# ayankele/dune-transformercvn

Hardware: AMD Instinct MI355X
Metric: events/sec (fwd+bwd) at batch=32, 8 prongs/event; fraction of MFMA roofline (higher is better)
Workload: dtype bf16; 1 GPU; TransformerCVN DenseNet [3,6,12,6,3] g32, fwd+loss+bwd, batch 32/GPU, 8 prongs/event, 3x400x280 maps, 6-layer encoder, dropout 0.1; global_batch=32, parallelism=dp1, precision=bf16

## Files before the change

dune-transformercvn_amd/csrc/densenet.hip:

```cpp
#include <string>
#include <vector>
#include <cstring>

#include "tcvn_rows.h"
#include <cstdlib>
#include "densenet_plan.h"

using namespace tcvn;

namespace {
constexpr float kEps = 1e-5f, kMom = 0.1f;
}

int DenseNetPlan::add_slot(const std::string& name, long numel, int kind) {
    slots.push_back({name, numel, kind});
    return (int)slots.size() - 1;
}
BnSlots DenseNetPlan::add_bn(const std::string& p, int c) {
    BnSlots s;
    s.w = add_slot(p + ".weight", c, TCVN_SLOT_PARAM);
    s.b = add_slot(p + ".bias", c, TCVN_SLOT_PARAM);
    s.rm = add_slot(p + ".running_mean", c, TCVN_SLOT_BUFFER);
    s.rv = add_slot(p + ".running_var", c, TCVN_SLOT_BUFFER);
    s.nbt = add_slot(p + ".num_batches_tracked", 1, TCVN_SLOT_COUNTER);
// ... 490 lines not shown
    const int mid = cfg.bn_size * cfg.growth, g = cfg.growth;
    char* D = s.ws + L.D[bi];
    char* Y = s.ws + L.Y[bi][l];
    double* bstatD = reinterpret_cast<double*>(s.ws + L.bstatD[bi]);
    double* bstatY = reinterpret_cast<double*>(s.ws + L.bstatY[bi][l]);
    long long* isumD = s.lf_on ? reinterpret_cast<long long*>(s.ws + L.isumD[bi]) : nullptr;
    long long* isumY = s.lf_on ? reinterpret_cast<long long*>(s.ws + L.isumY[bi][l]) : nullptr;
    int rc;
    ConvFwdArgs a = conv3_args(s, bi, l);
    Fwd1x1Args f1;
    const LayerPath p = path[bi][l] = layer_path(s, bi, l, a, f1);
    if (p.raw1x1) {
        if (s.lf_on && fr.isum) f1.lf = lf_link(s, ls.n1, isumD + 2 * fr.c0, 2L * bg.ld, fr.c0, fr.n, bstatD, M);
        else if ((rc = link_fresh(s, ls.n1, bi, fr))) return rc;
        f1.isum_out = isumY; f1.isum_stride = 2L * mid;
        if ((rc = fwd1x1_fused(f1, s.st))) return rc;
        if (!p.lf2 && (rc = link(s, ls.n2, f1.nblk, mid, 0, mid, bstatY, M, isumY, 2L * mid))) return rc;
    } else {
        if ((rc = link_fresh(s, ls.n1, bi, fr))) return rc;
        int nblk;
        if (L.XA[bi][l] >= 0) {
            const int cin8 = (int)round_up(ls.cin, 8);
            const Tab t1 = tab(s.ws, L, ls.n1);
            ActArgs act{D, bg.ld, M, ls.cin, t1.sc, t1.sh, data[ls.a1], s.ws + L.XA[bi][l], cin8};
            if ((rc = act_bf16(act, s.st))) return rc;
            const WkEntry& e = wk_find(ls.w1, 0, 1);
            GemmNtArgs ga{};
            ga.epi = EPI_FWD; ga.A = s.ws + L.XA[bi][l]; ga.lda = cin8; ga.K = cin8; ga.M = M; ga.N = mid;
            ga.Wfrag = s.ws + L.wk + e.off; ga.Kp = e.Kp; ga.zeros = s.ws + L.zeros; ga.bias = data[ls.b1];
            ga.Out = Y; ga.ldo = mid; ga.n_off = 0; ga.part = s.train ? s.part : nullptr; ga.nblk = gemm_nt_nblk(ga);
            if (p.fuse_ya) {
                ga.osc = a.sc; ga.osh = a.sh; ga.osl = a.sl; ga.Out = s.ws + L.YA[bi][l];
            }
            if ((rc = gemm_nt_bf16(ga, "k_gemm_nt_bf16<fwd1x1>", s.st))) return rc;
            nblk = ga.nblk;
        } else {
            ConvFwdArgs c1 = conv1_args(s, bi, l);
            c1.part = s.train ? s.part : nullptr; c1.nblk = conv_fwd_nblk(c1);
            if ((rc = conv_fwd(c1, s.st))) return rc;
            nblk = c1.nblk;
        }
        if ((rc = link(s, ls.n2, nblk, mid, 0, mid, bstatY, M))) return rc;
    }
    if (p.act_fused) a.act_fused = 1;
    else if (cfg.mode == MODE_BF16) {
        if (!p.fuse_ya) {
            ActArgs act{Y, mid, M, mid, a.sc, a.sh, a.sl, s.ws + L.YA[bi][l], mid};
            if ((rc = act_bf16(act, s.st))) return rc;
        }
        a.Aact = s.ws + L.YA[bi][l];
    }
    a.part = s.train ? s.part : nullptr;
    a.drop_p = s.train ? cfg.dropout : 0.f; a.seed = s.seed; a.stream_id = (uint32_t)(bi * 64 + l + 1);
    a.nblk = conv_fwd_nblk(a);
    if (p.lf2) {
        if (!a.act_fused) { fprintf(stderr, "tcvn: link-free norm2 without the in-LDS activation\n"); return -17; }
        a.lf = lf_link(s, ls.n2, isumY, 2L * mid, 0, mid, bstatY, M);
    }
    if (p.out_isum) { a.isum_out = isumD + 2 * ls.cin; a.isum_stride = 2L * bg.ld; }
    if (s.train && !L.KM[bi].empty()) a.keep_out = reinterpret_cast<uint32_t*>(s.ws + L.KM[bi][l]);
    if ((rc = conv_fwd(a, s.st))) return rc;
    fr = FreshStats{ls.cin, g, a.nblk, g, p.out_isum};
    return 0;
}

int DenseNetPlan::fwd_transition(const Step& s, int bi, FreshStats& fr) {
    const Layout& L = s.L;
    const BlockGeom& bg = blocks[bi];
    char* D = s.ws + L.D[bi];
    int rc;
    if ((rc = link_fresh(s, bg.has_trans ? bg.tn : nf, bi, fr))) return rc;
    if (!bg.has_trans) {
        const Tab t = tab(s.ws, L, nf);
        HeadPoolArgs a{cfg.mode, D, bg.ld, s.n, bg.H * bg.W, Cf, t.sc, t.sh, data[s_af], reinterpret_cast<float*>(s.ws + L.F)};
        return head_pool_fwd(a, s.st);
    }
    const BlockGeom& nb = blocks[bi + 1];
    fr = FreshStats{0, nb.C0, 0, bg.Ctot / 2, false};
    if (L.XP[bi] >= 0) {
        const Tab t = tab(s.ws, L, bg.tn);
        ActPoolArgs ap{D, bg.ld, s.n, bg.H, bg.W, bg.Ctot, t.sc, t.sh, data[bg.ta], s.ws + L.XP[bi], bg.ldp};
        if ((rc = cfg.mode == MODE_BF16 ? act_pool_bf16(ap, s.st) : act_pool_f32(ap, s.st))) return rc;
    }
    if (L.XP[bi] >= 0 && cfg.mode == MODE_BF16) {
        const WkEntry& ef = wk_find(bg.tw, 0, 1);
        GemmNtArgs ga{};
        ga.epi = EPI_FWD; ga.A = s.ws + L.XP[bi]; ga.lda = bg.ldp; ga.K = bg.ldp; ga.M = (long)s.n * nb.H * nb.W; ga.N = bg.Ctot / 2;
        ga.Wfrag = s.ws + L.wk + ef.off; ga.Kp = ef.Kp; ga.zeros = s.ws + L.zeros; ga.bias = data[bg.tb];
        ga.Out = s.ws + L.D[bi + 1]; ga.ldo = nb.ld; ga.n_off = 0; ga.part = s.train ? s.part : nullptr; ga.nblk = gemm_nt_nblk(ga);
        if ((rc = gemm_nt_bf16(ga, "k_gemm_nt_bf16<fwdtrans>", s.st))) return rc;
        fr.nblk = ga.nblk;
        return 0;
    }
    ConvFwdArgs a = trans_args(s, bi);
    a.part = s.train ? s.part : nullptr; a.nblk = conv_fwd_nblk(a);
    if ((rc = conv_fwd(a, s.st))) return rc;
    fr.nblk = a.nblk;
    return 0;
}

int DenseNetPlan::fwd_output(const Step& s, float* out, long out_ld) const {
    float* F = reinterpret_cast<float*>(s.ws + s.L.F);
    float* Z = reinterpret_cast<float*>(s.ws + s.L.Z);
    int rc;
    if ((rc = linear_fwd(F, Cf, data[s_wl], nullptr, Z, cfg.out_dim, s.n, cfg.out_dim, Cf, s.st))) return rc;
    float* hs = reinterpret_cast<float*>(s.ws + s.L.head_stat);
    RowsBnArgs r{};
    r.X = Z; r.ldx = cfg.out_dim; r.R = s.n; r.C = cfg.out_dim; r.gamma = data[nl.w]; r.beta = data[nl.b]; r.slope = data[s_al];
    r.running_mean = data[nl.rm]; r.running_var = data[nl.rv]; r.Y = out; r.ldy = out_ld;
    r.save_mean = hs; r.save_rstd = hs + cfg.out_dim; r.train = s.train; r.eps = kEps; r.momentum = kMom;
    r.drop_p = s.train ? cfg.dropout : 0.f; r.seed = s.seed; r.stream_id = 0x4000u;
    return rows_bn_fwd(r, s.st);
}

int DenseNetPlan::tap(int n, const char* name, long* off, int* tn, int* th, int* tw, int* tc, int* tld, int* tes) const {
    Layout L;
    layout(n, false, L);
    std::string s(name);
    *tn = n; *tes = esz;
    if ((s == "img" || s == "conv0") && stem_path.sparse && n == last_n) return -1;
    if (s == "img") { *off = L.img; *th = cfg.H; *tw = cfg.W; *tc = cfg.in_ch; *tld = cfg.in_ch; return 0; }
    if (s == "conv0") { *off = L.c0; *th = Hc; *tw = Wc; *tc = cfg.init_ch; *tld = cfg.init_ch; return 0; }
    if (s == "condense") { *off = L.F; *th = 1; *tw = 1; *tc = Cf; *tld = Cf; *tes = 4; return 0; }
    if (s == "raw:wk") { *tn = *th = *tw = 1; *off = L.wk; *tc = *tld = (int)(wk_bytes() / esz); return 0; }
    if (s == "raw:tabs") { *tn = *th = *tw = 1; *off = L.tabs; *tc = *tld = (int)tab_floats(); *tes = 4; return 0; }
    if (s.rfind("raw:ystat", 0) == 0) {
        int b = 0, l = 0;
        if (sscanf(s.c_str(), "raw:ystat%d.%d", &b, &l) != 2) return -1;
        b -= 1;
        if (b < 0 || b >= (int)blocks.size() || l < 0 || l >= blocks[b].L) return -1;
        *tn = *th = *tw = 1; *off = L.bstatY[b][l]; *tc = *tld = 2 * cfg.bn_size * cfg.growth; *tes = 8; return 0;
    }
    if (s.rfind("raw:isumy", 0) == 0) {
        int b = 0, l = 0;
        if (sscanf(s.c_str(), "raw:isumy%d.%d", &b, &l) != 2) return -1;
        b -= 1;
        if (b < 0 || b >= (int)blocks.size() || l < 0 || l >= blocks[b].L || L.isumY.empty() || n != last_n || !path[b][l].lf2) return -1;
        *tn = *th = *tw = 1; *off = L.isumY[b][l]; *tc = *tld = LF_REP * 2 * cfg.bn_size * cfg.growth; *tes = 8; return 0;
    }
    if (s.rfind("raw:bstat", 0) == 0) {
        const int b = atoi(s.c_str() + 9) - 1;
        if (s == "raw:bstat0") { *tn = *th = *tw = 1; *off = L.bstat0; *tc = *tld = cfg.init_ch * 2; *tes = 8; return 0; }
        if (b < 0 || b >= (int)blocks.size()) return -1;
        *tn = *th = *tw = 1; *off = L.bstatD[b]; *tc = *tld = blocks[b].ld * 2; *tes = 8; return 0;
    }
    if (s == "output_linear") { *off = L.Z; *th = 1; *tw = 1; *tc = *tld = cfg.out_dim; *tes = 4; return 0; }
    if (s.rfind("raw:grad", 0) == 0) {
        const int b = atoi(s.c_str() + 8) - 1;
        if (b < 0 || b >= (int)blocks.size()) return -1;
        Layout Lb;
        layout(n, true, Lb);
        *off = Lb.G[b]; *th = blocks[b].H; *tw = blocks[b].W; *tc = blocks[b].Ctot; *tld = blocks[b].ld; return 0;
    }
    if (s.rfind("raw:pq", 0) == 0) {
        const int b = atoi(s.c_str() + 6) - 1;
        if (b < 0 || b >= (int)blocks.size()) return -1;
        Layout Lb;
        layout(n, true, Lb);
        *tn = *th = *tw = 1; *off = Lb.pqD[b]; *tc = *tld = 2 * blocks[b].ld; *tes = 4; return 0;
    }
    if (s == "raw:dcondense") {
        Layout Lb;
        layout(n, true, Lb);
        *off = Lb.dF; *th = 1; *tw = 1; *tc = *tld = Cf; *tes = 4; return 0;
    }
    if (s.rfind("raw:du", 0) == 0) {
        const int b = atoi(s.c_str() + 6) - 1;
        if (b < 0 || b >= (int)blocks.size()) return -1;
        Layout Lb;
        layout(n, true, Lb);
        *off = Lb.du; *th = blocks[b].H; *tw = blocks[b].W; *tc = *tld = cfg.bn_size * cfg.growth; return 0;
    }
    if (s.rfind("raw:ey", 0) == 0) {
        int b = 0, l = 0;
        if (sscanf(s.c_str(), "raw:ey%d.%d", &b, &l) != 2) return -1;
        b -= 1;
        Layout Lb;
        layout(n, true, Lb);
        if (b < 0 || b >= (int)blocks.size() || l < 0 || l >= blocks[b].L || Lb.EY3[b].empty()) return -1;
        *off = Lb.EY3[b][l]; *th = blocks[b].H; *tw = blocks[b].W; *tc = *tld = 32; return 0;
    }
    if (s == "raw:head_stat") { *tn = *th = *tw = 1; *off = L.head_stat; *tc = *tld = 2 * cfg.out_dim; *tes = 4; return 0; }
    if (s.rfind("dense", 0) == 0) {
        const int b = atoi(s.c_str() + 5) - 1;
        if (b < 0 || b >= (int)blocks.size()) return -1;
        *off = L.D[b]; *th = blocks[b].H; *tw = blocks[b].W; *tc = blocks[b].Ctot; *tld = blocks[b].ld;
        return 0;
    }
    if (s.rfind("bottleneck", 0) == 0) {
        int b = 0, l = 0;
        if (sscanf(s.c_str(), "bottleneck%d.%d", &b, &l) != 2) return -1;
        b -= 1;
        if (b < 0 || b >= (int)blocks.size() || l < 0 || l >= blocks[b].L) return -1;
        for (const auto& pb : path)
            for (const LayerPath& p : pb) if (n == last_n && p.fuse_ya) return -1;
        *off = L.Y[b][l]; *th = blocks[b].H; *tw = blocks[b].W; *tc = cfg.bn_size * cfg.growth; *tld = *tc;
        return 0;
    }
    if (s.rfind("xa", 0) == 0 || s.rfind("ya", 0) == 0) {
        int b = 0, l = 0;
        if (sscanf(s.c_str() + 2, "%d.%d", &b, &l) != 2) return -1;
        b -= 1;
        if (b < 0 || b >= (int)blocks.size() || l < 0 || l >= blocks[b].L) return -1;
        const bool xa = s[0] == 'x';
        if ((xa && (L.XA[b].empty() || L.XA[b][l] < 0)) || (!xa && L.YA[b].empty())) return -1;
        if (n == last_n && (xa ? path[b][l].raw1x1 : path[b][l].act_fused)) return -1;
        *off = xa ? L.XA[b][l] : L.YA[b][l]; *th = blocks[b].H; *tw = blocks[b].W;
        *tc = xa ? blocks[b].layers[l].cin : cfg.bn_size * cfg.growth; *tld = xa ? (int)round_up(*tc, 8) : *tc;
        return 0;
    }
    return -1;
}

struct tcvn_densenet { DenseNetPlan plan; explicit tcvn_densenet(const tcvn_densenet_cfg& c) : plan(c) {} };

extern "C" {

int tcvn_version(void) { return 1; }
void tcvn_backward_overlap(int on) { tcvn::set_backward_overlap(on); }

int tcvn_densenet_create(const tcvn_densenet_cfg* cfg, tcvn_densenet** out) {
    if (!cfg || !out || cfg->n_blocks < 1 || cfg->n_blocks > 8) return -1;
    if (cfg->mode != TCVN_MODE_F32 && cfg->mode != TCVN_MODE_BF16) return -1;
    *out = new tcvn_densenet(*cfg);
    return 0;
}
void tcvn_densenet_destroy(tcvn_densenet* p) { delete p; }
int tcvn_densenet_num_slots(const tcvn_densenet* p) { return (int)p->plan.slots.size(); }
int tcvn_densenet_slot(const tcvn_densenet* p, int i, char* name, int cap, int64_t* numel, int* kind) {
    if (i < 0 || i >= (int)p->plan.slots.size()) return -1;
    const auto& s = p->plan.slots[i];
    if (name && cap > 0) { strncpy(name, s.name.c_str(), cap - 1); name[cap - 1] = 0; }
    if (numel) *numel = s.numel;
    if (kind) *kind = s.kind;
    return 0;
}
int tcvn_densenet_bind(tcvn_densenet* p, void* const* data, void* const* grad) { return p->plan.bind(data, grad); }
int64_t tcvn_densenet_workspace_bytes(const tcvn_densenet* p, int n_img, int with_backward) {
    Layout L;
    p->plan.layout(n_img, with_backward != 0, L);
    return L.total;
}
int tcvn_densenet_forward(tcvn_densenet* p, int n_img, const int32_t* coords, const float* values, int64_t nnz, int log_pixels,
                          float noise_std, float* out, int64_t out_ld, void* ws, int64_t ws_bytes, int train, uint64_t seed,
                          void* stream) {
    return p->plan.forward(n_img, coords, values, nnz, log_pixels, noise_std, out, out_ld, reinterpret_cast<char*>(ws), ws_bytes,
                           train, seed, reinterpret_cast<hipStream_t>(stream));
}
int tcvn_densenet_backward(tcvn_densenet* p, int n_img, const float* d_out, int64_t d_out_ld, void* ws, int64_t ws_bytes,
                           void* stream) {
    return p->plan.backward(n_img, d_out, d_out_ld, reinterpret_cast<char*>(ws), ws_bytes, reinterpret_cast<hipStream_t>(stream));
}
int tcvn_densenet_num_blocks(const tcvn_densenet* p) { return (int)p->plan.blocks.size(); }
int tcvn_densenet_backward_blocks(tcvn_densenet* p, int n_img, const float* d_out, int64_t d_out_ld, void* ws, int64_t ws_bytes,
                                  int block_hi, int block_lo, void* stream) {
    return p->plan.backward(n_img, d_out, d_out_ld, reinterpret_cast<char*>(ws), ws_bytes, reinterpret_cast<hipStream_t>(stream), block_hi,
                            block_lo);
}
int tcvn_densenet_tap(const tcvn_densenet* p, int n_img, const char* name, int64_t* byte_off, int* n, int* h, int* w, int* c,
                      int* ld, int* elem_bytes) {
    long off = 0;
    int rc = p->plan.tap(n_img, name, &off, n, h, w, c, ld, elem_bytes);
    *byte_off = off;
    return rc;
}

}
```

dune-transformercvn_amd/csrc/stem.hip:

```cpp
#include <cstdlib>
#include <type_traits>
#include "tcvn_ops.h"
#include "prof.h"

namespace tcvn {

namespace {

__global__ void k_stem_mark(const int* __restrict__ coords, long nnz, int n_img, int H, int W, int Hc, int Wc, int WW, uint32_t* __restrict__ act,
                            const float* __restrict__ bias, bf16* __restrict__ cline) {
    const long i = (long)blockIdx.x * blockDim.x + threadIdx.x;
    if (blockIdx.x == 0 && threadIdx.x < 64) cline[threadIdx.x] = f2bf(bias[threadIdx.x]);
    if (i >= nnz) return;
    const int img = coords[i * 3], y = coords[i * 3 + 1], x = coords[i * 3 + 2];
    if (img < 0 || img >= n_img || y < 0 || y >= H || x < 0 || x >= W) return;
    const int oy0 = max(0, (y - 2) >> 1), oy1 = min(Hc - 1, (y + 3) >> 1);
    const int ox0 = max(0, (x - 2) >> 1), ox1 = min(Wc - 1, (x + 3) >> 1);
    if (ox0 > ox1) return;
    const int w0 = ox0 >> 5, w1 = ox1 >> 5;
    const uint32_t m_lo = (w0 == w1 ? ((ox1 - ox0 + 1 >= 32) ? 0xffffffffu : ((1u << (ox1 - ox0 + 1)) - 1u)) : 0xffffffffu) << (ox0 & 31);
    const uint32_t m_hi = w0 == w1 ? 0u : (0xffffffffu >> (31 - (ox1 & 31)));
    for (int oy = oy0; oy <= oy1; ++oy) {
        uint32_t* row = act + ((long)img * Hc + oy) * WW;
        atomicOr(row + w0, m_lo);
        if (m_hi) atomicOr(row + w1, m_hi);
    }
}

__global__ __launch_bounds__(256) void k_pool0_bwd_vec(const Pool0BwdArgs a) {
    __shared__ double red[4][8][8][3];
    const bf16* X = reinterpret_cast<const bf16*>(a.X);
    const bf16* G = reinterpret_cast<const bf16*>(a.e.G);
    const bf16* D = reinterpret_cast<const bf16*>(a.e.X);
    bf16* DU = reinterpret_cast<bf16*>(a.DU);
    const int cpr = a.C >> 3;
    const int tid = threadIdx.x;
    const int c8 = tid % cpr;
    float sc[8], sh[8], sl[8], cP[8], cQ[8];
#pragma unroll
    for (int j = 0; j < 8; ++j) {
        sc[j] = a.sc[c8 * 8 + j]; sh[j] = a.sh[c8 * 8 + j]; sl[j] = a.sl[c8 * 8 + j];
        cP[j] = a.e.P[c8 * 8 + j]; cQ[j] = a.e.Q[c8 * 8 + j];
    }
    double s1[8], s2[8], s3[8];
#pragma unroll
    for (int j = 0; j < 8; ++j) { s1[j] = 0; s2[j] = 0; s3[j] = 0; }
    const int ppb = 256 / cpr;
    const long npix = (long)a.n_img * a.Hin * a.Win;
    for (long p = (long)blockIdx.x * ppb + tid / cpr; p < npix; p += (long)gridDim.x * ppb) {
        const int w = (int)(p % a.Win);
        const int h = (int)((p / a.Win) % a.Hin);
        const long img = p / ((long)a.Win * a.Hin);
        float dz[8] = {0, 0, 0, 0, 0, 0, 0, 0};
        const int ho_lo = max(0, (h - 1) / 2), ho_hi = min(a.Ho - 1, h / 2);
        const int wo_lo = max(0, (w - 1) / 2), wo_hi = min(a.Wo - 1, w / 2);
        for (int ho = ho_lo; ho <= ho_hi; ++ho)
            for (int wo = wo_lo; wo <= wo_hi; ++wo) {
                if (2 * ho > h || 2 * ho + 2 < h || 2 * wo > w || 2 * wo + 2 < w) continue;
                const long mo = (img * a.Ho + ho) * a.Wo + wo;
                const u16x8 gv = *reinterpret_cast<const u16x8*>(G + mo * a.e.ldg + c8 * 8);
                const u16x8 dv = *reinterpret_cast<const u16x8*>(D + mo * a.e.ldx + c8 * 8);
#pragma unroll
                for (int j = 0; j < 8; ++j) dz[j] += bf2f(gv[j]) + cP[j] * bf2f(dv[j]) + cQ[j];
            }
        const u16x8 xv = *reinterpret_cast<const u16x8*>(X + p * a.C + c8 * 8);
        u16x8 o;
#pragma unroll
        for (int j = 0; j < 8; ++j) {
            const float z = dz[j] * (1.0f / 9.0f);
            const float x = bf2f(xv[j]);
            const float u = fmaf(x, sc[j], sh[j]);
            const float du = u > 0.f ? z : sl[j] * z;
            s1[j] += du; s2[j] += (double)du * x; s3[j] += u > 0.f ? 0.f : z * u;
            o[j] = f2bf(sc[j] * du);
        }
        *reinterpret_cast<u16x8*>(DU + p * a.C + c8 * 8) = o;
    }
    const int lane = tid & 63, wave = tid >> 6;
#pragma unroll
    for (int j = 0; j < 8; ++j) {
#pragma unroll
        for (int o = 8; o < 64; o <<= 1) { s1[j] += __shfl_xor(s1[j], o); s2[j] += __shfl_xor(s2[j], o); s3[j] += __shfl_xor(s3[j], o); }
    }
    if (lane < 8) {
#pragma unroll
        for (int j = 0; j < 8; ++j) { red[wave][lane][j][0] = s1[j]; red[wave][lane][j][1] = s2[j]; red[wave][lane][j][2] = s3[j]; }
    }
    __syncthreads();
    if (tid < a.C) {
        const int ch = tid >> 3, j = tid & 7;
        double x = 0, y = 0, z = 0;
        for (int w = 0; w < 4; ++w)
            for (int l = ch; l < 8; l += cpr) { x += red[w][l][j][0]; y += red[w][l][j][1]; z += red[w][l][j][2]; }
        double* o = a.part + ((long)blockIdx.x * a.C + tid) * 3;
        o[0] = x; o[1] = y; o[2] = z;
    }
}

constexpr int SW_MAXC = 4;
template <typename T>
__global__ __launch_bounds__(256, 2) void k_stem_wgrad_sparse(const StemWgradArgs a) {
    __shared__ float wacc[49 * SW_MAXC][64];
    const int tid = threadIdx.x, lane = tid & 63;
    for (int i = tid; i < 49 * SW_MAXC * 64; i += 256) (&wacc[0][0])[i] = 0.f;
    __syncthreads();
    const T* img = reinterpret_cast<const T*>(a.img);
    const T* G = reinterpret_cast<const T*>(a.e.G);
    const T* X = reinterpret_cast<const T*>(a.e.X);
    const int n = lane;
    const bool nok = n < a.e.N;
    const float pn = nok ? a.e.P[n] : 0.f, qn = nok ? a.e.Q[n] : 0.f;
    float acc[49][3];
#pragma unroll
    for (int t = 0; t < 49; ++t) { acc[t][0] = 0.f; acc[t][1] = 0.f; acc[t][2] = 0.f; }
    const long gw = (long)blockIdx.x * 4 + (tid >> 6), nw = (long)gridDim.x * 4;
    int c_im = -1, c_y = 0, c_x = 0;
    if (gw < a.nnz) { c_im = a.coords[gw * 3]; c_y = a.coords[gw * 3 + 1]; c_x = a.coords[gw * 3 + 2]; }
    for (long hit = gw; hit < a.nnz; hit += nw) {
        const int im = __builtin_amdgcn_readfirstlane(c_im);
        const int y = __builtin_amdgcn_readfirstlane(c_y);
        const int x = __builtin_amdgcn_readfirstlane(c_x);
        if (hit + nw < a.nnz) { c_im = a.coords[(hit + nw) * 3]; c_y = a.coords[(hit + nw) * 3 + 1]; c_x = a.coords[(hit + nw) * 3 + 2]; }
        if (im < 0 || im >= a.n_img || y < 0 || y >= a.H || x < 0 || x >= a.W) continue;
        const T* px = img + (((long)im * a.H + y) * a.W + x) * a.Cpix;
        float v[3];
#pragma unroll
        for (int c = 0; c < 3; ++c) v[c] = c < a.Cpix ? to_f<T>(px[c]) : 0.f;
        auto taps = [&](auto pyc, auto pxc) {
            constexpr int PY = decltype(pyc)::value, PX = decltype(pxc)::value;
            constexpr int NY = PY ? 3 : 4, NX = PX ? 3 : 4;
            float gq[NY][NX], xq[NY][NX];
            bool okq[NY][NX];
#pragma unroll
            for (int iy = 0; iy < NY; ++iy)
#pragma unroll
                for (int ix = 0; ix < NX; ++ix) {
                    const int oy = (y + 3 - (PY + 2 * iy)) >> 1, ox = (x + 3 - (PX + 2 * ix)) >> 1;
                    okq[iy][ix] = ((unsigned)oy < (unsigned)a.Hc) & ((unsigned)ox < (unsigned)a.Wc) & nok;
                    const long p = okq[iy][ix] ? ((long)im * a.Hc + oy) * a.Wc + ox : 0;
                    gq[iy][ix] = to_f<T>(G[p * a.e.ldg + (nok ? n : 0)]);
                    xq[iy][ix] = to_f<T>(X[p * a.e.ldx + (nok ? n : 0)]);
                }
#pragma unroll
            for (int iy = 0; iy < NY; ++iy)
#pragma unroll
                for (int ix = 0; ix < NX; ++ix) {
                    const float eff = okq[iy][ix] ? gq[iy][ix] + pn * xq[iy][ix] + qn : 0.f;
                    constexpr int dummy = 0; (void)dummy;
                    const int t = (PY + 2 * iy) * 7 + (PX + 2 * ix);
#pragma unroll
                    for (int c = 0; c < 3; ++c) acc[t][c] = fmaf(v[c], eff, acc[t][c]);
                }
        };
        const int pyr = (y + 3) & 1, pxr = (x + 3) & 1;
        if (pyr == 0) { if (pxr == 0) taps(std::integral_constant<int, 0>{}, std::integral_constant<int, 0>{}); else taps(std::integral_constant<int, 0>{}, std::integral_constant<int, 1>{}); }
        else { if (pxr == 0) taps(std::integral_constant<int, 1>{}, std::integral_constant<int, 0>{}); else taps(std::integral_constant<int, 1>{}, std::integral_constant<int, 1>{}); }
    }
#pragma unroll
    for (int t = 0; t < 49; ++t)
#pragma unroll
        for (int c = 0; c < 3; ++c)
            if (c < a.Cpix) atomicAdd(&wacc[t * a.Cpix + c][n], acc[t][c]);
    __syncthreads();
    float* out = a.slab + (long)blockIdx.x * a.e.N * a.Kp;
    for (int i = tid; i < a.e.N * a.Kp; i += 256) {
        const int nn = i / a.Kp, k = i - nn * a.Kp;
        out[i] = k < 49 * a.Cpix ? wacc[k][nn] : 0.f;
    }
}



constexpr int PB_TH = 8, PB_TW = 32, PB_PH = PB_TH / 2 + 1, PB_PW = PB_TW / 2 + 1;
template <typename T> __device__ __forceinline__ void store8_g(T* p, const float v[8]);
template <> __device__ __forceinline__ void store8_g<float>(float* p, const float v[8]) {
    *reinterpret_cast<f32x4*>(p) = f32x4{v[0], v[1], v[2], v[3]};
    *reinterpret_cast<f32x4*>(p + 4) = f32x4{v[4], v[5], v[6], v[7]};
}
template <> __device__ __forceinline__ void store8_g<bf16>(bf16* p, const float v[8]) {
    u16x8 o;
#pragma unroll
    for (int j = 0; j < 8; ++j) o[j] = f2bf(v[j]);
    *reinterpret_cast<u16x8*>(p) = o;
}
template <typename T>
__global__ __launch_bounds__(256, 2) void k_pool0_bwd_tile(const Pool0BwdArgs a, int tiles_x, int tiles_y) {
    __shared__ __attribute__((aligned(16))) float effs[PB_PH * PB_PW * 64];
    __shared__ double red[4][8][8][3];
    const T* X = reinterpret_cast<const T*>(a.X);
    const T* G = reinterpret_cast<const T*>(a.e.G);
    const T* D = reinterpret_cast<const T*>(a.e.X);
    T* DU = reinterpret_cast<T*>(a.DU);
    const int tid = threadIdx.x, c8 = tid & 7;
    __shared__ __attribute__((aligned(16))) float tabs[5][64];
    __shared__ uint32_t actw[PB_TH];
    const int WW = (a.Win + 31) >> 5;
    if (tid < 64) { tabs[0][tid] = a.sc[tid]; tabs[1][tid] = a.sh[tid]; tabs[2][tid] = a.sl[tid]; tabs[3][tid] = a.e.P[tid]; tabs[4][tid] = a.e.Q[tid]; }
    auto tab8 = [&](int which, float (&v)[8]) {
        const float4 x0 = *reinterpret_cast<const float4*>(&tabs[which][c8 * 8]), x1 = *reinterpret_cast<const float4*>(&tabs[which][c8 * 8 + 4]);
        v[0] = x0.x; v[1] = x0.y; v[2] = x0.z; v[3] = x0.w; v[4] = x1.x; v[5] = x1.y; v[6] = x1.z; v[7] = x1.w;
    };
    float s1[8], s2[8], s3[8];
#pragma unroll
    for (int j = 0; j < 8; ++j) { s1[j] = 0; s2[j] = 0; s3[j] = 0; }
    const long ntiles = (long)a.n_img * tiles_x * tiles_y;
    for (long tile = blockIdx.x; tile < ntiles; tile += gridDim.x) {
        const int tx = (int)(tile % tiles_x), ty = (int)((tile / tiles_x) % tiles_y);
        const long img = tile / ((long)tiles_x * tiles_y);
        const int h0 = ty * PB_TH, w0 = tx * PB_TW, ho0 = h0 / 2 - 1, wo0 = w0 / 2 - 1;
        __syncthreads();
        if (tid < PB_TH) actw[tid] = (a.act != nullptr && h0 + tid < a.Hin) ? a.act[(img * a.Hin + h0 + tid) * WW + tx] : 0xffffffffu;
        {
            constexpr int NP1 = (PB_PH * PB_PW * 8 + 255) / 256;
            float gv[NP1][8], dv[NP1][8];
            bool in[NP1];
#pragma unroll
            for (int k = 0; k < NP1; ++k) {
                const int i = tid + 256 * k, pp = i >> 3, py = pp / PB_PW, px = pp - py * PB_PW, ho = ho0 + py, wo = wo0 + px;
                in[k] = (i < PB_PH * PB_PW * 8) & (ho >= 0) & (ho < a.Ho) & (wo >= 0) & (wo < a.Wo);
                const long mo = in[k] ? (img * a.Ho + ho) * a.Wo + wo : img * a.Ho * a.Wo;
                load8<T>(G + mo * a.e.ldg + c8 * 8, gv[k]);
                load8<T>(D + mo * a.e.ldx + c8 * 8, dv[k]);
            }
            float cP[8], cQ[8];
            tab8(3, cP); tab8(4, cQ);
#pragma unroll
            for (int k = 0; k < NP1; ++k) {
                const int i = tid + 256 * k, pp = i >> 3;
                if (i < PB_PH * PB_PW * 8) {
                    float e8[8];
#pragma unroll
                    for (int j = 0; j < 8; ++j) e8[j] = in[k] ? gv[k][j] + cP[j] * dv[k][j] + cQ[j] : 0.f;
                    float4* o = reinterpret_cast<float4*>(effs + pp * 64 + c8 * 8);
                    o[0] = make_float4(e8[0], e8[1], e8[2], e8[3]); o[1] = make_float4(e8[4], e8[5], e8[6], e8[7]);
                }
            }
        }
        __syncthreads();
#pragma unroll 1
        for (int k = 0; k < PB_TH * PB_TW / 128; ++k) {
            const int bi = (tid >> 3) + 32 * k, by = bi / (PB_TW / 2), bx = bi - by * (PB_TW / 2);
            const int h = h0 + 2 * by, w = w0 + 2 * bx;
            float xv[4][8];
            bool ok[4], live[4];
            const uint32_t aw0 = actw[2 * by] >> (2 * bx), aw1 = actw[2 * by + 1] >> (2 * bx);
#pragma unroll
            for (int t = 0; t < 4; ++t) {
                const int hh = h + (t >> 1), ww = w + (t & 1);
                ok[t] = (hh < a.Hin) & (ww < a.Win);
                live[t] = ok[t] & ((((t >> 1) ? aw1 : aw0) >> (t & 1)) & 1u);
                const long p = ok[t] ? (img * a.Hin + hh) * a.Win + ww : img * a.Hin * a.Win;
                const T* src = (a.act == nullptr || live[t]) ? X + p * a.C + c8 * 8 : reinterpret_cast<const T*>(a.cline) + c8 * 8;
                load8<T>(src, xv[t]);
            }
            float e[4][8], sc[8], sh[8], sl[8];
            tab8(0, sc); tab8(1, sh); tab8(2, sl);
#pragma unroll
            for (int t = 0; t < 4; ++t) {
                const float4* e4 = reinterpret_cast<const float4*>(effs + ((by + (t >> 1)) * PB_PW + bx + (t & 1)) * 64 + c8 * 8);
                const float4 x0 = e4[0], x1 = e4[1];
                e[t][0] = x0.x; e[t][1] = x0.y; e[t][2] = x0.z; e[t][3] = x0.w; e[t][4] = x1.x; e[t][5] = x1.y; e[t][6] = x1.z; e[t][7] = x1.w;
            }
#pragma unroll
            for (int t = 0; t < 4; ++t) {
                float o[8];
#pragma unroll
                for (int j = 0; j < 8; ++j) {
                    const float lower = e[2][j] + e[3][j], right = e[1][j] + e[3][j];
                    const float dzs = t == 0 ? lower + e[0][j] + e[1][j] : t == 1 ? right : t == 2 ? lower : e[3][j];
                    const float z = ok[t] ? dzs * (1.0f / 9.0f) : 0.f;
                    const float x = xv[t][j];
                    const float u = fmaf(x, sc[j], sh[j]);
                    const float du = u > 0.f ? z : sl[j] * z;
                    s1[j] += du; s2[j] = fmaf(du, x, s2[j]); s3[j] += u > 0.f ? 0.f : z * u;
                    o[j] = sc[j] * du;
                }
                if (live[t]) store8_g<T>(DU + ((img * a.Hin + h + (t >> 1)) * a.Win + w + (t & 1)) * a.C + c8 * 8, o);
            }
        }
    }
    const int lane = tid & 63, wave = tid >> 6;
#pragma unroll
    for (int j = 0; j < 8; ++j) {
        double d1 = (double)s1[j], d2 = (double)s2[j], d3 = (double)s3[j];
#pragma unroll
        for (int o = 8; o < 64; o <<= 1) { d1 += __shfl_xor(d1, o); d2 += __shfl_xor(d2, o); d3 += __shfl_xor(d3, o); }
        if (lane < 8) { red[wave][lane][j][0] = d1; red[wave][lane][j][1] = d2; red[wave][lane][j][2] = d3; }
    }
    __syncthreads();
    if (tid < 64) {
        const int ch = tid >> 3, j = tid & 7;
        double x = 0, y = 0, z = 0;
        for (int w = 0; w < 4; ++w) { x += red[w][ch][j][0]; y += red[w][ch][j][1]; z += red[w][ch][j][2]; }
        double* o = a.part + ((long)blockIdx.x * a.C + tid) * 3;
        o[0] = x; o[1] = y; o[2] = z;
    }
}

constexpr int ST_TH = 8, ST_TW = 16;
constexpr int ST_PR = 2 * ST_TH + 5, ST_PW = 40;
constexpr int ST_CP = 72;

#ifdef TCVN_DEBUG_KNOBS
__global__ __launch_bounds__(256, 2) void k_stem_fwd_bf16(const ConvFwdArgs g, int n_img, int tiles_x, int tiles_y) {
    __shared__ __attribute__((aligned(16))) unsigned short patch[2][ST_PR * ST_PW * 4];
    __shared__ __attribute__((aligned(16))) unsigned short ctile[ST_TH * ST_TW * ST_CP];
    __shared__ double red[4][64][2];
    const int tid = threadIdx.x, lane = tid & 63, wave = tid >> 6;
    const int r = lane & 31, h = lane >> 5;
    const bf16* __restrict__ img = reinterpret_cast<const bf16*>(g.A);
    const bf16* __restrict__ Wk = reinterpret_cast<const bf16*>(g.Wk);
    bf16* __restrict__ Out = reinterpret_cast<bf16*>(g.Out);
    const int Hin = g.Hin, Win = g.Win, Ho = g.H, Wo = g.W;
    const long ntiles = (long)n_img * tiles_x * tiles_y;

    bf16x8_t bw[2][14];
#pragma unroll
    for (int nt = 0; nt < 2; ++nt)
#pragma unroll
        for (int s = 0; s < 14; ++s) {
            u16x8 w;
#pragma unroll
            for (int i = 0; i < 8; ++i) {
// ... 130 lines not shown
#pragma unroll
    for (int ct = 0; ct < 2; ++ct)
#pragma unroll
        for (int k = 0; k < 16; ++k) { bias[ct][k] = g.bias[ct * 32 + (k & 3) + 8 * (k >> 2) + 4 * h]; f1[ct][k] = 0.f; f2[ct][k] = 0.f; }
    for (int i = tid; i < 2 * ST_PR * ST_PW * 4; i += 256) (&patch[0][0])[i] = 0;

    constexpr int NE = ST_PR * 37 * 3, PER = (NE + 255) / 256;
    int e_pr[PER], e_pc[PER];
#pragma unroll
    for (int k = 0; k < PER; ++k) {
        const int i = tid + 256 * k;
        const int pr = i / 111, e = i - pr * 111, px = e / 3, c = e - px * 3;
        e_pr[k] = i < NE ? pr : -100000;
        e_pc[k] = px * 4 + c;
    }
    auto load_patch = [&](unsigned tile, unsigned short (&v)[PER]) {
        const unsigned trow = tile / tiles_x;
        const int tx = (int)(tile - trow * tiles_x), ty = (int)(trow % tiles_y);
        const long n = trow / tiles_y;
        const int iy0 = 2 * ty * ST_TH - 3, ix0 = 2 * tx * ST_TW - 3;
        const bf16* base = img + ((n * Hin + iy0) * (long)Win + ix0) * 3;
#pragma unroll
        for (int k = 0; k < PER; ++k) {
            const int px = e_pc[k] >> 2, c = e_pc[k] & 3;
            const int iy = iy0 + e_pr[k], ix = ix0 + px;
            const bool ok = ((unsigned)iy < (unsigned)Hin) & ((unsigned)ix < (unsigned)Win);
            const unsigned short x = *(ok ? base + (e_pr[k] * Win + px) * 3 + c : img);
            v[k] = ok ? x : (unsigned short)0;
        }
    };
    auto store_patch = [&](int buf, const unsigned short (&v)[PER]) {
#pragma unroll
        for (int k = 0; k < PER; ++k)
            if (e_pr[k] >= 0) patch[buf][e_pr[k] * (ST_PW * 4) + e_pc[k]] = v[k];
    };

    unsigned short pv[PER];
    unsigned tile = blockIdx.x;
    __syncthreads();
    if (tile < ntiles) { load_patch(tile, pv); store_patch(0, pv); }
    __syncthreads();
    int cur = 0;
    const int oy_l = 2 * wave + (r >> 4), ox_l = r & 15;
    for (; tile < ntiles; tile += gridDim.x, cur ^= 1) {
        const bool more = tile + gridDim.x < ntiles;
        if (more) load_patch(tile + gridDim.x, pv);
        f32x16 acc[2];
#pragma unroll
        for (int ct = 0; ct < 2; ++ct)
#pragma unroll
            for (int k = 0; k < 16; ++k) acc[ct][k] = 0.f;
        const unsigned short* pb = &patch[cur][0];
#pragma unroll
        for (int s = 0; s < 14; ++s) {
            const int gq = 2 * s + h, ky = gq >> 2, q4 = gq & 3;
            const bf16x8_t b = *reinterpret_cast<const bf16x8_t*>(pb + ((2 * oy_l + ky) * ST_PW + 2 * ox_l + 2 * q4) * 4);
            const bf16x8_t w0 = *reinterpret_cast<const bf16x8_t*>(&wl[(s * 64 + lane) * 8]);
            const bf16x8_t w1 = *reinterpret_cast<const bf16x8_t*>(&wl[((14 + s) * 64 + lane) * 8]);
            acc[0] = __builtin_amdgcn_mfma_f32_32x32x16_bf16(w0, b, acc[0], 0, 0, 0);
            acc[1] = __builtin_amdgcn_mfma_f32_32x32x16_bf16(w1, b, acc[1], 0, 0, 0);
        }
        const unsigned trow = tile / tiles_x;
        const int tx = (int)(tile - trow * tiles_x), ty = (int)(trow % tiles_y);
        const long n = trow / tiles_y;
        const int oy0 = ty * ST_TH, ox0 = tx * ST_TW;
        const float vm = ((oy0 + oy_l < Ho) & (ox0 + ox_l < Wo)) ? 1.f : 0.f;
        unsigned short* cp = &ctile[(oy_l * ST_TW + ox_l) * ST_CP + 4 * h];
#pragma unroll
        for (int ct = 0; ct < 2; ++ct)
#pragma unroll
            for (int gq = 0; gq < 4; ++gq) {
                u16x4 o;
#pragma unroll
                for (int j = 0; j < 4; ++j) {
                    const int k = gq * 4 + j;
                    o[j] = f2bf(acc[ct][k] + bias[ct][k]);
                    const float x = bf2f(o[j]) * vm;
                    f1[ct][k] += x; f2[ct][k] = fmaf(x, x, f2[ct][k]);
                }
                *reinterpret_cast<u16x4*>(cp + ct * 32 + gq * 8) = o;
            }
        if (more) store_patch(cur ^ 1, pv);
        __syncthreads();
#pragma unroll
        for (int k = 0; k < 4; ++k) {
            const int idx = tid + 256 * k, p = idx >> 3, c8 = idx & 7;
            const int py = p >> 4, px = p & 15;
            if ((oy0 + py < Ho) & (ox0 + px < Wo))
                *reinterpret_cast<u16x8*>(Out + ((n * Ho + oy0 + py) * (long)Wo + ox0 + px) * g.ldo + c8 * 8) =
                    *reinterpret_cast<const u16x8*>(&ctile[p * ST_CP + c8 * 8]);
        }
        __syncthreads();
    }
    if (g.part != nullptr) {
#pragma unroll
        for (int ct = 0; ct < 2; ++ct)
#pragma unroll
            for (int k = 0; k < 16; ++k) {
                double a = (double)f1[ct][k], b = (double)f2[ct][k];
#pragma unroll
                for (int o = 1; o < 32; o <<= 1) { a += __shfl_xor(a, o); b += __shfl_xor(b, o); }
                if (r == 0) { const int c = ct * 32 + (k & 3) + 8 * (k >> 2) + 4 * h; red[wave][c][0] = a; red[wave][c][1] = b; }
            }
        __syncthreads();
        if (tid < 64) {
            double a = 0, b = 0;
#pragma unroll
            for (int w = 0; w < 4; ++w) { a += red[w][tid][0]; b += red[w][tid][1]; }
            g.part[((long)blockIdx.x * 64 + tid) * 2] = a;
            g.part[((long)blockIdx.x * 64 + tid) * 2 + 1] = b;
        }
    }
}

}

int pool0_bwd_vec_grid(int n_img, int Hin, int Win) {
    const long g = ((long)n_img * Hin * Win + 31) / 32;
    return (int)(g < 2048 ? g : 2048);
}
bool pool0_bwd_vec_ok(const Pool0BwdArgs& a) {
    if (a.mode == MODE_F32) return conv3x3_tile_enabled() && a.C == 64 && (a.e.ldg & 7) == 0 && (a.e.ldx & 7) == 0;
    return a.mode == MODE_BF16 && (a.C == 8 || a.C == 16 || a.C == 32 || a.C == 64) && (a.e.ldg & 7) == 0 && (a.e.ldx & 7) == 0;
}
int pool0_bwd_vec(const Pool0BwdArgs& a, hipStream_t st) {
    if (!pool0_bwd_vec_ok(a)) return -2;
    if (a.nblk != pool0_bwd_vec_grid(a.n_img, a.Hin, a.Win)) return -3;
    static const bool old = TCVN_KNOB_SET("TCVN_POOL0_BWD_FLAT");
    if (a.mode == MODE_F32) {
        hipLaunchKernelGGL(k_pool0_bwd_tile<float>, dim3(a.nblk), dim3(256), 0, st, a, cdiv(a.Win, PB_TW), cdiv(a.Hin, PB_TH));
        TCVN_LAUNCH_CHECK();
        return 0;
    }
    if (a.C == 64 && !old) {
        hipLaunchKernelGGL(k_pool0_bwd_tile<bf16>, dim3(a.nblk), dim3(256), 0, st, a, cdiv(a.Win, PB_TW), cdiv(a.Hin, PB_TH));
        TCVN_LAUNCH_CHECK();
        return 0;
    }
    hipLaunchKernelGGL(k_pool0_bwd_vec, dim3(a.nblk), dim3(256), 0, st, a);
    TCVN_LAUNCH_CHECK();
    return 0;
}

int stem_mark(const int* coords, long nnz, int n_img, int H, int W, int Hc, int Wc, uint32_t* act, const float* bias, void* cline, hipStream_t st) {
    const int WW = stem_act_words(Wc);
    TCVN_CHECK(hipMemsetAsync(act, 0, (size_t)n_img * Hc * WW * 4, st));
    hipLaunchKernelGGL(k_stem_mark, dim3(cdiv(nnz > 0 ? nnz : 1, 256)), dim3(256), 0, st, coords, nnz, n_img, H, W, Hc, Wc, WW, act, bias, reinterpret_cast<bf16*>(cline));
    TCVN_LAUNCH_CHECK();
    return 0;
}

int stem_wgrad_sparse(const StemWgradArgs& a, float* dWk, hipStream_t st) {
    if (a.Cpix > 3 || a.e.N > 64 || a.Kp < 49 * a.Cpix) return -2;
    const int nb = 512;
    if ((long)nb * a.e.N * a.Kp * 4 > a.slab_bytes) return -3;
    {
        ProfScope ps("k_stem_wgrad_sparse", 2.0 * a.nnz * 12.25 * a.Cpix * a.e.N, 0.0, st);
        if (a.mode == MODE_F32) hipLaunchKernelGGL(k_stem_wgrad_sparse<float>, dim3(nb), dim3(256), 0, st, a);
        else hipLaunchKernelGGL(k_stem_wgrad_sparse<bf16>, dim3(nb), dim3(256), 0, st, a);
        TCVN_LAUNCH_CHECK();
    }
    return slab_reduce(a.slab, nb, (long)a.e.N * a.Kp, dWk, st);
}


bool stem_fwd_ok(const ConvFwdArgs& a) {
    return conv3x3_tile_enabled() && a.mode == MODE_BF16 && a.amode == A_STEM && a.C == 3 && a.N == 64 && a.K == 147 && a.Kp >= 147 &&
           a.ldo == 64 && a.n_off == 0 && a.Hin == 2 * a.H && a.Win == 2 * a.W && a.M % (a.H * a.W) == 0 &&
           (reinterpret_cast<uintptr_t>(a.Out) & 15) == 0;
}
int stem_fwd_nblk(const ConvFwdArgs& a) {
    const long nt = (long)(a.M / (a.H * a.W)) * cdiv(a.W, ST_TW) * cdiv(a.H, ST_TH);
    return (int)(nt < 512 ? nt : 512);
}
int stem_fwd_bf16(const ConvFwdArgs& a, hipStream_t st) {
    const int n_img = a.M / (a.H * a.W);
    ProfScope ps("k_stem_fwd_bf16", 2.0 * a.M * (double)a.N * a.K, (double)a.M * 2.0 * (a.N + 4.0 * a.C), st);
#ifdef TCVN_DEBUG_KNOBS
    static const bool v1 = TCVN_KNOB_SET("TCVN_STEM_FWD_V1");
    if (v1) {
        hipLaunchKernelGGL(k_stem_fwd_bf16, dim3(stem_fwd_nblk(a)), dim3(256), 0, st, a, n_img, cdiv(a.W, ST_TW), cdiv(a.H, ST_TH));
        TCVN_LAUNCH_CHECK();
        return 0;
    }
#endif
    hipLaunchKernelGGL(k_stem_fwd2_bf16, dim3(stem_fwd_nblk(a)), dim3(256), 0, st, a, n_img, cdiv(a.W, ST_TW), cdiv(a.H, ST_TH));
    TCVN_LAUNCH_CHECK();
    return 0;
}

}
```

Before: 1795 events/s.

## Restructure sparse stem wgrad into per-parity waves with contiguous chunks

The sparse stem weight-gradient kernel now gives each block a contiguous chunk of hits. Each of its four waves handles one (y,x) parity class, with a compile-time tap count instead of a 49-tap accumulator that branches per hit. Lanes load 64 coordinates at once, ballot the hits that match their class, and process two hits at a time to overlap gathers. Results are written to shared memory without atomics, and the grid is sized from nnz with a 3-blocks-per-CU launch bound. A debug entry point and raw:du0/pq0 tensor introspection are also added. Wave load can become unbalanced when hit parities are skewed.

```diff
diff --git a/dune-transformercvn_amd/csrc/densenet.hip b/dune-transformercvn_amd/csrc/densenet.hip
--- a/dune-transformercvn_amd/csrc/densenet.hip
+++ b/dune-transformercvn_amd/csrc/densenet.hip
@@ -666,6 +666,13 @@
         layout(n, true, Lb);
         *off = Lb.G[b]; *th = blocks[b].H; *tw = blocks[b].W; *tc = blocks[b].Ctot; *tld = blocks[b].ld; return 0;
     }
+    if (s == "raw:du0" || s == "raw:pq0") {
+        if (stem_path.sparse && n == last_n) return -1;
+        Layout Lb;
+        layout(n, true, Lb);
+        if (s == "raw:du0") { *off = Lb.du0; *th = Hc; *tw = Wc; *tc = *tld = cfg.init_ch; return 0; }
+        *tn = *th = *tw = 1; *off = Lb.pq0; *tc = *tld = 2 * cfg.init_ch; *tes = 4; return 0;
+    }
     if (s.rfind("raw:pq", 0) == 0) {
         const int b = atoi(s.c_str() + 6) - 1;
         if (b < 0 || b >= (int)blocks.size()) return -1;
diff --git a/dune-transformercvn_amd/csrc/stem.hip b/dune-transformercvn_amd/csrc/stem.hip
--- a/dune-transformercvn_amd/csrc/stem.hip
+++ b/dune-transformercvn_amd/csrc/stem.hip
@@ -97,70 +97,104 @@
     }
 }
 
-constexpr int SW_MAXC = 4;
-template <typename T>
-__global__ __launch_bounds__(256, 2) void k_stem_wgrad_sparse(const StemWgradArgs a) {
-    __shared__ float wacc[49 * SW_MAXC][64];
-    const int tid = threadIdx.x, lane = tid & 63;
-    for (int i = tid; i < 49 * SW_MAXC * 64; i += 256) (&wacc[0][0])[i] = 0.f;
-    __syncthreads();
+constexpr int SW_CHUNK_MIN = 64;
+constexpr int SW_WG_PER_CU = 3;
+constexpr int SW_GRID_MAX = 256 * SW_WG_PER_CU;
+int stem_wgrad_grid(long nnz) {
+    const long want = (nnz + SW_CHUNK_MIN - 1) / SW_CHUNK_MIN;
+    return (int)(want < 1 ? 1 : want > SW_GRID_MAX ? SW_GRID_MAX : want);
+}
+
+template <typename T, int PY, int PX>
+__device__ __forceinline__ void stem_wgrad_class(const StemWgradArgs& a, float (*wacc)[64], long h0, long h1, int lane) {
+    constexpr int NY = PY ? 3 : 4, NX = PX ? 3 : 4, NT = NY * NX;
     const T* img = reinterpret_cast<const T*>(a.img);
     const T* G = reinterpret_cast<const T*>(a.e.G);
     const T* X = reinterpret_cast<const T*>(a.e.X);
     const int n = lane;
     const bool nok = n < a.e.N;
+    const int nc = nok ? n : 0;
     const float pn = nok ? a.e.P[n] : 0.f, qn = nok ? a.e.Q[n] : 0.f;
-    float acc[49][3];
-#pragma unroll
-    for (int t = 0; t < 49; ++t) { acc[t][0] = 0.f; acc[t][1] = 0.f; acc[t][2] = 0.f; }
-    const long gw = (long)blockIdx.x * 4 + (tid >> 6), nw = (long)gridDim.x * 4;
-    int c_im = -1, c_y = 0, c_x = 0;
-    if (gw < a.nnz) { c_im = a.coords[gw * 3]; c_y = a.coords[gw * 3 + 1]; c_x = a.coords[gw * 3 + 2]; }
-    for (long hit = gw; hit < a.nnz; hit += nw) {
-        const int im = __builtin_amdgcn_readfirstlane(c_im);
-        const int y = __builtin_amdgcn_readfirstlane(c_y);
-        const int x = __builtin_amdgcn_readfirstlane(c_x);
-        if (hit + nw < a.nnz) { c_im = a.coords[(hit + nw) * 3]; c_y = a.coords[(hit + nw) * 3 + 1]; c_x = a.coords[(hit + nw) * 3 + 2]; }
-        if (im < 0 || im >= a.n_img || y < 0 || y >= a.H || x < 0 || x >= a.W) continue;
-        const T* px = img + (((long)im * a.H + y) * a.W + x) * a.Cpix;
-        float v[3];
+    float acc[NT][3];
+#pragma unroll
+    for (int t = 0; t < NT; ++t) { acc[t][0] = 0.f; acc[t][1] = 0.f; acc[t][2] = 0.f; }
+    auto request = [&](bool live, int im, int y, int x, float (&gq)[NT], float (&xq)[NT], unsigned& ok, float (&v)[3]) {
+        const T* px = img + (live ? (((long)im * a.H + y) * a.W + x) * a.Cpix : 0);
 #pragma unroll
         for (int c = 0; c < 3; ++c) v[c] = c < a.Cpix ? to_f<T>(px[c]) : 0.f;
-        auto taps = [&](auto pyc, auto pxc) {
-            constexpr int PY = decltype(pyc)::value, PX = decltype(pxc)::value;
-            constexpr int NY = PY ? 3 : 4, NX = PX ? 3 : 4;
-            float gq[NY][NX], xq[NY][NX];
-            bool okq[NY][NX];
-#pragma unroll
-            for (int iy = 0; iy < NY; ++iy)
-#pragma unroll
-                for (int ix = 0; ix < NX; ++ix) {
-                    const int oy = (y + 3 - (PY + 2 * iy)) >> 1, ox = (x + 3 - (PX + 2 * ix)) >> 1;
-                    okq[iy][ix] = ((unsigned)oy < (unsigned)a.Hc) & ((unsigned)ox < (unsigned)a.Wc) & nok;
-                    const long p = okq[iy][ix] ? ((long)im * a.Hc + oy) * a.Wc + ox : 0;
-                    gq[iy][ix] = to_f<T>(G[p * a.e.ldg + (nok ? n : 0)]);
-                    xq[iy][ix] = to_f<T>(X[p * a.e.ldx + (nok ? n : 0)]);
-                }
-#pragma unroll
-            for (int iy = 0; iy < NY; ++iy)
-#pragma unroll
-                for (int ix = 0; ix < NX; ++ix) {
-                    const float eff = okq[iy][ix] ? gq[iy][ix] + pn * xq[iy][ix] + qn : 0.f;
-                    constexpr int dummy = 0; (void)dummy;
-                    const int t = (PY + 2 * iy) * 7 + (PX + 2 * ix);
-#pragma unroll
-                    for (int c = 0; c < 3; ++c) acc[t][c] = fmaf(v[c], eff, acc[t][c]);
-                }
-        };
-        const int pyr = (y + 3) & 1, pxr = (x + 3) & 1;
-        if (pyr == 0) { if (pxr == 0) taps(std::integral_constant<int, 0>{}, std::integral_constant<int, 0>{}); else taps(std::integral_constant<int, 0>{}, std::integral_constant<int, 1>{}); }
-        else { if (pxr == 0) taps(std::integral_constant<int, 1>{}, std::integral_constant<int, 0>{}); else taps(std::integral_constant<int, 1>{}, std::integral_constant<int, 1>{}); }
-    }
-#pragma unroll
-    for (int t = 0; t < 49; ++t)
-#pragma unroll
-        for (int c = 0; c < 3; ++c)
-            if (c < a.Cpix) atomicAdd(&wacc[t * a.Cpix + c][n], acc[t][c]);
+        ok = 0u;
+#pragma unroll
+        for (int iy = 0; iy < NY; ++iy)
+#pragma unroll
+            for (int ix = 0; ix < NX; ++ix) {
+                const int t = iy * NX + ix;
+                const int oy = (y + 3 - (PY + 2 * iy)) >> 1, ox = (x + 3 - (PX + 2 * ix)) >> 1;
+                const bool in = live & ((unsigned)oy < (unsigned)a.Hc) & ((unsigned)ox < (unsigned)a.Wc) & nok;
+                ok |= (in ? 1u : 0u) << t;
+                const long p = in ? ((long)im * a.Hc + oy) * a.Wc + ox : 0;
+                gq[t] = to_f<T>(G[p * a.e.ldg + nc]);
+                xq[t] = to_f<T>(X[p * a.e.ldx + nc]);
+            }
+    };
+    auto add = [&](const float (&gq)[NT], const float (&xq)[NT], unsigned ok, const float (&v)[3]) {
+#pragma unroll
+        for (int t = 0; t < NT; ++t) {
+            const float eff = ((ok >> t) & 1u) ? gq[t] + pn * xq[t] + qn : 0.f;
+#pragma unroll
+            for (int c = 0; c < 3; ++c) acc[t][c] = fmaf(v[c], eff, acc[t][c]);
+        }
+    };
+    auto load_coords = [&](long base, int& im, int& y, int& x) {
+        const long h = base + lane;
+        im = -1; y = 0; x = 0;
+        if (h < h1) { im = a.coords[h * 3]; y = a.coords[h * 3 + 1]; x = a.coords[h * 3 + 2]; }
+    };
+    int c_im, c_y, c_x;
+    load_coords(h0, c_im, c_y, c_x);
+    for (long base = h0; base < h1; base += 64) {
+        const int l_im = c_im, l_y = c_y, l_x = c_x;
+        load_coords(base + 64, c_im, c_y, c_x);
+        const bool mine = l_im >= 0 && l_im < a.n_img && (unsigned)l_y < (unsigned)a.H && (unsigned)l_x < (unsigned)a.W &&
+                          ((l_y + 3) & 1) == PY && ((l_x + 3) & 1) == PX;
+        unsigned long long m = __ballot(mine);
+        while (m) {
+            const int l0 = __ffsll((long long)m) - 1;
+            m &= m - 1;
+            const bool two = m != 0;
+            const int l1 = two ? __ffsll((long long)m) - 1 : l0;
+            m &= m - 1;
+            float g0[NT], x0[NT], v0[3], g1[NT], x1[NT], v1[3];
+            unsigned ok0, ok1;
+            request(true, __builtin_amdgcn_readlane(l_im, l0), __builtin_amdgcn_readlane(l_y, l0), __builtin_amdgcn_readlane(l_x, l0), g0, x0, ok0, v0);
+            request(two, __builtin_amdgcn_readlane(l_im, l1), __builtin_amdgcn_readlane(l_y, l1), __builtin_amdgcn_readlane(l_x, l1), g1, x1, ok1, v1);
+            add(g0, x0, ok0, v0);
+            add(g1, x1, ok1, v1);
+        }
+    }
+#pragma unroll
+    for (int iy = 0; iy < NY; ++iy)
+#pragma unroll
+        for (int ix = 0; ix < NX; ++ix) {
+            const int tap = (PY + 2 * iy) * 7 + PX + 2 * ix;
+#pragma unroll
+            for (int c = 0; c < 3; ++c)
+                if (c < a.Cpix) wacc[tap * a.Cpix + c][n] = acc[iy * NX + ix][c];
+        }
+}
+
+template <typename T>
+__global__ __launch_bounds__(256, SW_WG_PER_CU) void k_stem_wgrad_sparse(const StemWgradArgs a) {
+    __shared__ float wacc[49 * 3][64];
+    const int tid = threadIdx.x, lane = tid & 63;
+    const int wave = __builtin_amdgcn_readfirstlane(tid >> 6);
+    const long chunk = (a.nnz + gridDim.x - 1) / gridDim.x;
+    const long lo = (long)blockIdx.x * chunk, h0 = lo < a.nnz ? lo : a.nnz, h1 = h0 + chunk < a.nnz ? h0 + chunk : a.nnz;
+    switch (wave) {
+        case 0: stem_wgrad_class<T, 0, 0>(a, wacc, h0, h1, lane); break;
+        case 1: stem_wgrad_class<T, 0, 1>(a, wacc, h0, h1, lane); break;
+        case 2: stem_wgrad_class<T, 1, 0>(a, wacc, h0, h1, lane); break;
+        default: stem_wgrad_class<T, 1, 1>(a, wacc, h0, h1, lane); break;
+    }
     __syncthreads();
     float* out = a.slab + (long)blockIdx.x * a.e.N * a.Kp;
     for (int i = tid; i < a.e.N * a.Kp; i += 256) {
@@ -168,7 +202,6 @@
         out[i] = k < 49 * a.Cpix ? wacc[k][nn] : 0.f;
     }
 }
-
 
 
 constexpr int PB_TH = 8, PB_TW = 32, PB_PH = PB_TH / 2 + 1, PB_PW = PB_TW / 2 + 1;
@@ -605,7 +638,7 @@
 
 int stem_wgrad_sparse(const StemWgradArgs& a, float* dWk, hipStream_t st) {
     if (a.Cpix > 3 || a.e.N > 64 || a.Kp < 49 * a.Cpix) return -2;
-    const int nb = 512;
+    const int nb = stem_wgrad_grid(a.nnz);
     if ((long)nb * a.e.N * a.Kp * 4 > a.slab_bytes) return -3;
     {
         ProfScope ps("k_stem_wgrad_sparse", 2.0 * a.nnz * 12.25 * a.Cpix * a.e.N, 0.0, st);
@@ -615,6 +648,18 @@
     }
     return slab_reduce(a.slab, nb, (long)a.e.N * a.Kp, dWk, st);
 }
+
+#ifdef TCVN_DEBUG_KNOBS
+extern "C" int tcvn_debug_stem_wgrad(int mode, const int* coords, long nnz, const void* img, int n_img, int H, int W, int Cpix, const void* G,
+                                     const void* X, const float* P, const float* Q, int N, int Hc, int Wc, int Kp, float* slab, long slab_bytes,
+                                     float* dWk, void* stream, int* nblk) {
+    if (nblk != nullptr) *nblk = stem_wgrad_grid(nnz);
+    if (dWk == nullptr) return 0;
+    const EffSrc e{G, N, X, N, 0, N, P, Q, 0.f, 0, 0};
+    const StemWgradArgs a{coords, nnz, img, n_img, H, W, Cpix, e, Hc, Wc, Kp, slab, slab_bytes, mode};
+    return stem_wgrad_sparse(a, dWk, reinterpret_cast<hipStream_t>(stream));
+}
+#endif
 
 
 bool stem_fwd_ok(const ConvFwdArgs& a) {
```

Measured after the change: 1803 events/s, median of 6. No clear change (+0.5%).
